# vvvm23/distributed-pytorch-cookbook

Hardware: AMD Instinct MI355X
Metric: tokens/sec (node) GPT-2 training per recipe (DDP/FSDP/PP) at 1/2/4/8 MI355X (higher is better)
Workload: dtype bf16; 1 GPU; model=gpt2-small, global_batch=64, seq_len=1024, parallelism=dp1, recipe=main-ddp.py, reduce_dtype=fp32, pp_comm_dtype=fp32, step_graph=True

## Files before the change

distributed_pytorch_cookbook_amd/ops/csrc/attention.hip:

```cpp
#include "common.h"

#include <cstdlib>
#include <type_traits>

namespace dpc {

struct AttnArgs {
  const void* q; const void* k; const void* v;
  void* o;
  float* lse;
  const unsigned char* pad;
  const void* dout;
  void* dq; void* dk; void* dv;
  float* delta;
  long long ld_qkv, ld_o, ld_dqkv;
  int N, S, H;
  float scale;
  int causal;
  int hd;
  int order;
};

constexpr int KT = 64;
constexpr int QB = 128;
constexpr int NSLOT = 4;
constexpr float LOG2E = 1.4426950408889634f;

template <int HD>
struct AT {
  static_assert(HD == 32 || HD == 64 || HD == 128, "head_dim 32, 64 or 128");
  static constexpr int TILE = KT * HD;
  static constexpr int NPW = HD / 32;
  static constexpr int NST = HD / 16;
  static constexpr int NDT = HD / 32;
};

typedef short4_t __attribute__((address_space(3))) * lds4_t;
typedef __attribute__((address_space(3))) void* lds_void_t;

__device__ __forceinline__ int aswz(int prow) {
  const int a = (prow >> 1) & 7;
  return a ^ ((a & 1) << 2);
}
template <int HD>
__device__ __forceinline__ int toff(int row, int chunk) {
  const int e = row * HD + chunk * 8;
  const int prow = e >> 6, pch = (e >> 3) & 7;
  return (prow << 6) + ((pch ^ aswz(prow)) << 3);
}

__device__ __forceinline__ void dma16(__amdgpu_buffer_rsrc_t rs, int voff, const void* lds) {
  const unsigned la = (unsigned)(uintptr_t)(lds_void_t)lds;
  asm volatile("s_mov_b32 m0, %2\n\ts_nop 0\n\tbuffer_load_dwordx4 %0, %1, 0 offen lds"
               :
               : "v"(voff), "s"(rs), "s"(la)
               : "memory", "m0");
}
__device__ __forceinline__ void dma4(__amdgpu_buffer_rsrc_t rs, int voff, const void* lds) {
  const unsigned la = (unsigned)(uintptr_t)(lds_void_t)lds;
  asm volatile("s_mov_b32 m0, %2\n\ts_nop 0\n\tbuffer_load_dword %0, %1, 0 offen lds"
               :
               : "v"(voff), "s"(rs), "s"(la)
               : "memory", "m0");
}
template <int N>
__device__ __forceinline__ void vm_wait() {
  asm volatile("s_waitcnt vmcnt(%0)" ::"n"(N) : "memory");
}
template <int N>
__device__ __forceinline__ void pin_loaded(const bf16x8 (&x)[N]) {
#pragma unroll
  for (int i = 0; i < N; ++i) asm volatile("" ::"v"(x[i]));
}
__device__ __forceinline__ void pin_loaded(float x) { asm volatile("" ::"v"(x)); }

__device__ __forceinline__ void ring_barrier() {
  __builtin_amdgcn_s_barrier();
  asm volatile("" ::: "memory");
}

__device__ __forceinline__ __amdgpu_buffer_rsrc_t rows_rsrc(const void* base, unsigned ld_bytes, int row0, int S,
                                                           bool valid) {
  const unsigned span = (unsigned)S * ld_bytes;
  const unsigned off = (unsigned)row0 * ld_bytes;
  const unsigned nrec = __builtin_amdgcn_readfirstlane((valid && off < span) ? span - off : 0u);
  return __builtin_amdgcn_make_buffer_rsrc((void*)((const char*)base + off), 0, nrec, 0x00020000);
}

template <int HD>
__device__ __forceinline__ void dma_voff(int (&v)[AT<HD>::NPW], long long ld, int wid, int lane) {
#pragma unroll
  for (int i = 0; i < AT<HD>::NPW; ++i) {
    const int prow = 8 * (wid * AT<HD>::NPW + i) + (lane >> 3);
    const int e = prow * 64 + (((lane & 7) ^ aswz(prow)) << 3);
    const int row = e / HD, chunk = (e % HD) >> 3;
    v[i] = (int)((long long)row * ld * 2 + chunk * 16);
  }
}

template <int HD>
__device__ __forceinline__ void tile_dma(const bf16_t* base, long long ld, int row0, int S, bool valid,
                                         const int (&v)[AT<HD>::NPW], bf16_t* lds, int wid) {
  const __amdgpu_buffer_rsrc_t rs = rows_rsrc(base, (unsigned)(ld * 2), row0, S, valid);
#pragma unroll
  for (int i = 0; i < AT<HD>::NPW; ++i) dma16(rs, v[i], lds + (wid * AT<HD>::NPW + i) * 512);
}

template <int HD>
__device__ __forceinline__ bf16x8 row_frag(const bf16_t* lds, int row0, int st, int lane) {
  return *reinterpret_cast<const bf16x8*>(lds + toff<HD>(row0 + (lane & 31), 2 * st + (lane >> 5)));
}

template <int HD>
__device__ __forceinline__ bf16x8 tr_frag(const bf16_t* lds, int r0, int s, int c0, int lane) {
  const int h = lane >> 5, g2 = (lane >> 4) & 1, i16 = lane & 15, q = i16 >> 2, p = i16 & 3;
  const int row = r0 + 16 * s + 4 * h + q;
  const int col = c0 + 16 * g2 + 4 * p;
  const bf16_t* a0 = lds + toff<HD>(row, col >> 3) + (col & 7);
  const bf16_t* a1 = lds + toff<HD>(row + 8, col >> 3) + (col & 7);
  short4_t lo = __builtin_amdgcn_ds_read_tr16_b64_v4i16((lds4_t)a0);
  short4_t hi = __builtin_amdgcn_ds_read_tr16_b64_v4i16((lds4_t)a1);
  typedef short short8_t __attribute__((ext_vector_type(8)));
  short8_t s8 = {lo[0], lo[1], lo[2], lo[3], hi[0], hi[1], hi[2], hi[3]};
  return __builtin_bit_cast(bf16x8, s8);
}

__device__ __forceinline__ bf16x8 acc_frag(const floatx16& x, int s) {
  uint4 u;
  u.x = pack2bf(x[8 * s + 0], x[8 * s + 1]);
  u.y = pack2bf(x[8 * s + 2], x[8 * s + 3]);
  u.z = pack2bf(x[8 * s + 4], x[8 * s + 5]);
  u.w = pack2bf(x[8 * s + 6], x[8 * s + 7]);
  return __builtin_bit_cast(bf16x8, u);
}

__device__ __forceinline__ int acc_row(int r, int lane) { return (r & 3) + 8 * (r >> 2) + 4 * (lane >> 5); }

__device__ __forceinline__ void store_pair16(bf16_t* row, int g, int hh, uint2 wa, uint2 wb) {
  const auto s0 = __builtin_amdgcn_permlane32_swap(wa.x, wb.x, false, false);
  const auto s1 = __builtin_amdgcn_permlane32_swap(wa.y, wb.y, false, false);
  *reinterpret_cast<uint4*>(row + 8 * g + 8 * hh) = make_uint4(s0[0], s1[0], s0[1], s1[1]);
}

__device__ __forceinline__ float fast_exp2(float x) { return __builtin_amdgcn_exp2f(x); }

__device__ __forceinline__ float max3f(float a, float b, float c) { return fmaxf(fmaxf(a, b), c); }

__device__ __forceinline__ unsigned long long pad_bits(const unsigned char* pad, int k0, int S, int lane) {
  if (!pad) return 0ull;
  const int k = k0 + lane;
  return __ballot(k < S && pad[k] != 0);
}

__device__ __forceinline__ bf16x8 load_row8(const bf16_t* p) {
  return *reinterpret_cast<const bf16x8*>(p);
}

#define MFMA32(a, b, c) __builtin_amdgcn_mfma_f32_32x32x16_bf16((a), (b), (c), 0, 0, 0)

__device__ __forceinline__ void scale16(floatx16& x, float a) {
#pragma unroll
  for (int i = 0; i < 16; ++i) asm volatile("v_mul_f32 %0, %0, %1" : "+v"(x[i]) : "v"(a));
}

template <int K>
__device__ __forceinline__ void zero_if_gt(floatx16& x, int r, int v) {
  asm volatile("v_cmp_lt_i32_e32 vcc, %1, %2\n\tv_cndmask_b32_e64 %0, %0, 0, vcc"
               : "+v"(x[r])
               : "n"(K), "v"(v)
               : "vcc");
}

#define DPC_RS_MUL(i) "v_mul_f32 %" #i ", %" #i ", %16\n\t"
__device__ __forceinline__ void scale16_if(floatx16& x, float a, unsigned long long up) {
  asm volatile(
      "s_cmp_eq_u64 %17, 0\n\t"
      "s_cbranch_scc1 .Ldpc_rs%=\n\t"
      "s_nop 7\n\ts_nop 7\n\t"
      DPC_RS_MUL(0) DPC_RS_MUL(1) DPC_RS_MUL(2) DPC_RS_MUL(3) DPC_RS_MUL(4) DPC_RS_MUL(5) DPC_RS_MUL(6)
      DPC_RS_MUL(7) DPC_RS_MUL(8) DPC_RS_MUL(9) DPC_RS_MUL(10) DPC_RS_MUL(11) DPC_RS_MUL(12)
      DPC_RS_MUL(13) DPC_RS_MUL(14) DPC_RS_MUL(15)
      "s_nop 7\n"
      ".Ldpc_rs%=:"
      : "+v"(x[0]), "+v"(x[1]), "+v"(x[2]), "+v"(x[3]), "+v"(x[4]), "+v"(x[5]), "+v"(x[6]), "+v"(x[7]),
        "+v"(x[8]), "+v"(x[9]), "+v"(x[10]), "+v"(x[11]), "+v"(x[12]), "+v"(x[13]), "+v"(x[14]), "+v"(x[15])
      : "v"(a), "s"(up)
      : "scc");
}
#undef DPC_RS_MUL

#define DPC_RS_MUL(i) "v_mul_f32 %" #i ", %" #i ", %17\n\t"
__device__ __forceinline__ float rescale16_if(floatx16& x, float& m, float& l, float mx, unsigned long long up) {
  float a;
  asm volatile(
      "s_cmp_eq_u64 %20, 0\n\t"
      "s_cbranch_scc1 .Ldpc_ru%=\n\t"
      "s_nop 7\n\ts_nop 7\n\t"
      "v_max_f32 %17, %16, %19\n\t"
      "v_sub_f32 %16, %16, %17\n\t"
      "v_exp_f32 %16, %16\n\t"
      "s_nop 0\n\t"
      "v_swap_b32 %16, %17\n\t"
      "v_mul_f32 %18, %18, %17\n\t"
      DPC_RS_MUL(0) DPC_RS_MUL(1) DPC_RS_MUL(2) DPC_RS_MUL(3) DPC_RS_MUL(4) DPC_RS_MUL(5) DPC_RS_MUL(6)
      DPC_RS_MUL(7) DPC_RS_MUL(8) DPC_RS_MUL(9) DPC_RS_MUL(10) DPC_RS_MUL(11) DPC_RS_MUL(12)
      DPC_RS_MUL(13) DPC_RS_MUL(14) DPC_RS_MUL(15)
      "s_nop 7\n"
      ".Ldpc_ru%=:"
      : "+v"(x[0]), "+v"(x[1]), "+v"(x[2]), "+v"(x[3]), "+v"(x[4]), "+v"(x[5]), "+v"(x[6]), "+v"(x[7]),
        "+v"(x[8]), "+v"(x[9]), "+v"(x[10]), "+v"(x[11]), "+v"(x[12]), "+v"(x[13]), "+v"(x[14]), "+v"(x[15]),
        "+v"(m), "=&v"(a), "+v"(l)
      : "v"(mx), "s"(up)
      : "scc");
  return a;
}
#undef DPC_RS_MUL

__device__ __forceinline__ void zero16(floatx16& x) {
#pragma unroll
  for (int i = 0; i < 16; ++i) x[i] = 0.f;
}

__device__ __forceinline__ int g7_local_attn(int b, int grid) {
  const int xcd = b & 7, q = grid >> 3, r = grid & 7;
  return (xcd < r ? xcd * (q + 1) : r * (q + 1) + (xcd - r) * q) + (b >> 3);
}
__device__ __forceinline__ void work_order1(int nblk, int& bh, int& i) {
  const int nbh = gridDim.x / nblk;
  i = blockIdx.x / nbh;
  bh = blockIdx.x - i * nbh;
}
__device__ __forceinline__ void xcd_work(int nblk, int& bh, int& i) {
  const int b = blockIdx.x, nwg = gridDim.x, xcd = b & 7, q = nwg >> 3, r = nwg & 7;
  const int t = (xcd < r ? xcd * (q + 1) : r * (q + 1) + (xcd - r) * q) + (b >> 3);
  bh = t / nblk;
  i = t - bh * nblk;
}

template <int HD, int OCC>
__global__ __launch_bounds__(256, OCC) void attn_fwd_kernel(AttnArgs p) {
  using A = AT<HD>;
  __shared__ __attribute__((aligned(16))) bf16_t smem[NSLOT * 2 * A::TILE];
  const int S = p.S, H = p.H;
  const int nqb = (S + QB - 1) / QB;
  int bh, bi;
  xcd_work(nqb, bh, bi);
  const int qb = nqb - 1 - bi;
  const int n = bh / H, h = bh % H;
  const int lane = threadIdx.x & 63, hh = lane >> 5;
  const int wid = __builtin_amdgcn_readfirstlane(threadIdx.x >> 6);
  const int q0 = qb * QB + wid * 32;
  const int q = q0 + (lane & 31);
  const long long tok0 = (long long)n * S;
  const bf16_t* Q = static_cast<const bf16_t*>(p.q) + h * HD;
  const bf16_t* K = static_cast<const bf16_t*>(p.k) + tok0 * p.ld_qkv + h * HD;
  const bf16_t* V = static_cast<const bf16_t*>(p.v) + tok0 * p.ld_qkv + h * HD;

  bf16x8 qf[A::NST];
#pragma unroll
  for (int st = 0; st < A::NST; ++st)
    qf[st] = q < S ? load_row8(Q + (tok0 + q) * p.ld_qkv + 16 * st + 8 * hh) : bf16x8{};
  pin_loaded(qf);
  const float c = p.scale * LOG2E;
  const int kend = p.causal ? min(S, qb * QB + QB) : S;
  const int ntiles = (kend + KT - 1) / KT;
  const int last_w = p.causal ? min(ntiles - 1, max(0, min(q0 + 31, S - 1)) / KT) : ntiles - 1;
  const unsigned char* pad = p.pad ? p.pad + (long long)n * S : nullptr;

  int dv[A::NPW];
  dma_voff<HD>(dv, p.ld_qkv, wid, lane);
  auto issue = [&](int t) {
    bf16_t* st = smem + (t % NSLOT) * 2 * A::TILE;
    const bool valid = t < ntiles;
    tile_dma<HD>(K, p.ld_qkv, t * KT, S, valid, dv, st, wid);
    tile_dma<HD>(V, p.ld_qkv, t * KT, S, valid, dv, st + A::TILE, wid);
  };
  auto qk = [&](floatx16 (&s)[2], const bf16_t* lk) {
#pragma unroll
    for (int kb = 0; kb < 2; ++kb) {
      zero16(s[kb]);
#pragma unroll
      for (int st = 0; st < A::NST; ++st)
        s[kb] = MFMA32(row_frag<HD>(lk, kb * 32, st, lane), qf[st], s[kb]);
    }
  };

  float m = -INFINITY, l = 0.f;
  floatx16 o[A::NDT];
#pragma unroll
  for (int d = 0; d < A::NDT; ++d) zero16(o[d]);

  issue(0);
  issue(1);
  issue(2);
  vm_wait<4 * A::NPW>();
  ring_barrier();
  auto step = [&](int t, floatx16 (&sc)[2], floatx16 (&sn)[2]) {
    vm_wait<2 * A::NPW>();
    ring_barrier();
    issue(t + 3);
    const bf16_t* lkn = smem + ((t + 1) % NSLOT) * 2 * A::TILE;
    const bf16_t* lv = smem + (t % NSLOT) * 2 * A::TILE + A::TILE;
    if (t > last_w) return;
    const int kt0 = t * KT;
    const bool need_mask = (p.causal && kt0 + KT - 1 > q0) || (kt0 + KT > S) || pad;
    if (need_mask) {
      const unsigned long long pm = pad_bits(pad, kt0, S, lane);
      const int lim = (p.causal ? min(q, S - 1) : S - 1) - kt0;
#pragma unroll
      for (int kb = 0; kb < 2; ++kb)
#pragma unroll
        for (int r = 0; r < 16; ++r) {
          const int kl = kb * 32 + acc_row(r, lane);
          if (kl > lim || ((pm >> kl) & 1ull)) sc[kb][r] = -INFINITY;
        }
    }
    float mq[4];
#pragma unroll
    for (int q4 = 0; q4 < 4; ++q4) {
      const floatx16& sq = sc[q4 >> 1];
      const int r0 = (q4 & 1) * 8;
      float v = max3f(sq[r0], sq[r0 + 1], sq[r0 + 2]);
      v = max3f(v, sq[r0 + 3], sq[r0 + 4]);
      v = max3f(v, sq[r0 + 5], sq[r0 + 6]);
      mq[q4] = fmaxf(v, sq[r0 + 7]);
    }
    float mx = fmaxf(max3f(mq[0], mq[1], mq[2]), mq[3]);
    mx = fmaxf(mx, __shfl_xor(mx, 32, 64)) * c;
    if (__ballot(mx > m + 8.f)) {
      const float mn = fmaxf(m, mx);
      const float alpha = (mn == -INFINITY) ? 1.f : fast_exp2(m - mn);
      m = mn;
      l *= alpha;
#pragma unroll
      for (int d = 0; d < A::NDT; ++d) scale16(o[d], alpha);
    }
    const float nmu = (m == -INFINITY) ? 0.f : -m;
    qk(sn, lkn);
    float ls = 0.f;
    bf16x8 pb[2][2];
#pragma unroll
    for (int kb = 0; kb < 2; ++kb) {
#pragma unroll
      for (int r = 0; r < 16; ++r) {
        const float e = fast_exp2(fmaf(sc[kb][r], c, nmu));
        sc[kb][r] = e;
        ls += e;
      }
      pb[kb][0] = acc_frag(sc[kb], 0);
      pb[kb][1] = acc_frag(sc[kb], 1);
    }
    l += ls;
#pragma unroll
    for (int kb = 0; kb < 2; ++kb)
#pragma unroll
      for (int ss = 0; ss < 2; ++ss)
#pragma unroll
        for (int d = 0; d < A::NDT; ++d)
          o[d] = MFMA32(tr_frag<HD>(lv, kb * 32, ss, d * 32, lane), pb[kb][ss], o[d]);
  };
  floatx16 s0[2], s1[2];
  qk(s0, smem);
  for (int t = 0; t < ntiles; t += 2) {
    step(t, s0, s1);
    if (t + 1 < ntiles) step(t + 1, s1, s0);
  }
  vm_wait<0>();

  l += __shfl_xor(l, 32, 64);
  if (q < S) {
    const float inv = l > 0.f ? 1.f / l : 0.f;
    bf16_t* O = static_cast<bf16_t*>(p.o) + (tok0 + q) * p.ld_o + h * HD;
#pragma unroll
    for (int d = 0; d < A::NDT; ++d)
#pragma unroll
      for (int g = 0; g < 4; g += 2) {
        uint2 wa, wb;
        wa.x = pack2bf(o[d][4 * g + 0] * inv, o[d][4 * g + 1] * inv);
        wa.y = pack2bf(o[d][4 * g + 2] * inv, o[d][4 * g + 3] * inv);
        wb.x = pack2bf(o[d][4 * g + 4] * inv, o[d][4 * g + 5] * inv);
        wb.y = pack2bf(o[d][4 * g + 6] * inv, o[d][4 * g + 7] * inv);
        store_pair16(O + d * 32, g, hh, wa, wb);
      }
    if (hh == 0) {
      const float lse = (l > 0.f) ? (m + log2f(l)) / LOG2E : INFINITY;
      p.lse[(long long)bh * S + q] = lse;
    }
  }
}

struct PairItem {
  int bh, blk0, blk1, len0, len;
};

template <int HD, int OCC>
__global__ __launch_bounds__(256, OCC) void attn_fwd2_kernel(AttnArgs p, int nitems) {
  using A = AT<HD>;
  __shared__ __attribute__((aligned(16))) bf16_t smem[NSLOT * 2 * A::TILE];
  const int S = p.S, H = p.H;
  const int nqb = (S + QB - 1) / QB;
  const int npr = (nqb + 1) / 2;
  const int grid = gridDim.x;
  const int local = g7_local_attn(blockIdx.x, grid);
  const int lane = threadIdx.x & 63, hh = lane >> 5;
  const int wid = __builtin_amdgcn_readfirstlane(threadIdx.x >> 6);
  auto ntiles_of = [&](int qb) {
    const int kend = p.causal ? min(S, qb * QB + QB) : S;
    return (kend + KT - 1) / KT;
  };
  auto item = [&](int k) {
    PairItem it;
    const int id = local + k * grid;
    it.bh = id / npr;
    const int pr = id - it.bh * npr;
    it.blk0 = nqb - 1 - pr;
    it.blk1 = pr;
    it.len0 = 1 + ntiles_of(it.blk0);
    it.len = it.len0 + (it.blk1 != it.blk0 ? 1 + ntiles_of(it.blk1) : 0);
    return it;
  };
  const int nmine = local < nitems ? (nitems - local + grid - 1) / grid : 0;
  if (nmine == 0) return;
  int total = 0;
  for (int k = 0; k < nmine; ++k) total += item(k).len;

  int dv[A::NPW];
  dma_voff<HD>(dv, p.ld_qkv, wid, lane);
  int is_k = 0, is_off = 0;
  PairItem is_it = item(0);
  long long is_hoff = 0;
  auto enter = [&]() {
    const int n = is_it.bh / H, h = is_it.bh - n * H;
    is_hoff = (long long)n * S * p.ld_qkv + h * HD;
  };
  enter();
  auto issue_next = [&](int e) {
    bf16_t* st = smem + (e % NSLOT) * 2 * A::TILE;
    const bool valid = is_k < nmine;
    const bool second = is_off >= is_it.len0;
    const int i = is_off - (second ? is_it.len0 : 0);
    if (i == 0 || !valid) {
      const bf16_t* base = static_cast<const bf16_t*>(p.q) + is_hoff;
      const int r0 = (second ? is_it.blk1 : is_it.blk0) * QB;
      tile_dma<HD>(base, p.ld_qkv, r0, S, valid, dv, st, wid);
// ... 216 lines not shown
      const int r0 = (second ? is_it.blk1 : is_it.blk0) * QB;
      tile_dma<HD>(base, p.ld_qkv, r0, S, valid, dv, st, wid);
      tile_dma<HD>(base, p.ld_qkv, r0 + KT, S, valid, dv, st + A::TILE, wid);
    } else {
      const bf16_t* K = static_cast<const bf16_t*>(p.k) + is_hoff;
      const bf16_t* V = static_cast<const bf16_t*>(p.v) + is_hoff;
      tile_dma<HD>(K, p.ld_qkv, (i - 1) * KT, S, true, dv, st, wid);
      tile_dma<HD>(V, p.ld_qkv, (i - 1) * KT, S, true, dv, st + A::TILE, wid);
    }
    if (valid && ++is_off == is_it.len) {
      is_off = 0;
      if (++is_k < nmine) {
        is_it = item(is_k);
        enter();
      }
    }
  };
  auto sync = [&](int e) {
    vm_wait<2 * A::NPW>();
    ring_barrier();
    issue_next(e + 3);
  };
  auto slot = [&](int e) -> const bf16_t* { return smem + (e % NSLOT) * 2 * A::TILE; };

  const float c = p.scale * LOG2E;
  bf16x8 qf[A::NST];
  float m = -INFINITY, l = 0.f;
  floatx16 o[A::NDT];
  int q0 = 0, q = 0, last_w = 0;
  int bh = 0, h = 0, n = 0;
  const unsigned char* pad = nullptr;

  auto qk = [&](floatx16 (&s)[2], const bf16_t* lk) {
#pragma unroll
    for (int kb = 0; kb < 2; ++kb) {
      zero16(s[kb]);
#pragma unroll
      for (int st = 0; st < A::NST; ++st) s[kb] = MFMA32(row_frag<HD>(lk, kb * 32, st, lane), qf[st], s[kb]);
    }
  };
  auto finish = [&]() {
    l += __shfl_xor(l, 32, 64);
    if (q < S) {
      const float inv = l > 0.f ? __builtin_amdgcn_rcpf(l) : 0.f;
      bf16_t* O = static_cast<bf16_t*>(p.o) + (long long)n * S * p.ld_o + h * HD + q * (int)p.ld_o;
#pragma unroll
      for (int d = 0; d < A::NDT; ++d)
#pragma unroll
        for (int g = 0; g < 4; g += 2) {
          uint2 wa, wb;
          wa.x = pack2bf(o[d][4 * g + 0] * inv, o[d][4 * g + 1] * inv);
          wa.y = pack2bf(o[d][4 * g + 2] * inv, o[d][4 * g + 3] * inv);
          wb.x = pack2bf(o[d][4 * g + 4] * inv, o[d][4 * g + 5] * inv);
          wb.y = pack2bf(o[d][4 * g + 6] * inv, o[d][4 * g + 7] * inv);
          store_pair16(O + d * 32, g, hh, wa, wb);
        }
      if (hh == 0) p.lse[(long long)bh * S + q] = (l > 0.f) ? (m + log2f(l)) / LOG2E : INFINITY;
    }
  };
  auto tile = [&](auto gen, int e, int t, floatx16 (&sc)[2], floatx16 (&sn)[2]) {
    constexpr bool GEN = decltype(gen)::value;
    const bf16_t* ls = slot(e);
    const bf16_t* lv = ls + A::TILE;
    const int kt0 = t * KT;
    if constexpr (GEN) {
      const bool need_mask = (p.causal && kt0 + KT - 1 > q0) || (kt0 + KT > S) || pad;
      if (need_mask) {
        const int limh = (p.causal ? min(q, S - 1) : S - 1) - kt0 - 4 * hh;
        const unsigned long long pm = pad_bits(pad, kt0, S, lane) >> (4 * hh);
#pragma unroll
        for (int kb = 0; kb < 2; ++kb) {
          const unsigned pk = (unsigned)(pm >> (32 * kb));
#pragma unroll
          for (int r = 0; r < 16; ++r) {
            const int kc = kb * 32 + (r & 3) + 8 * (r >> 2);
            const bool masked = (kc > limh) || ((pk >> ((r & 3) + 8 * (r >> 2))) & 1u);
            if (masked) sc[kb][r] = -INFINITY;
          }
        }
      }
    }
    float mq[4];
#pragma unroll
    for (int q4 = 0; q4 < 4; ++q4) {
      const floatx16& sq = sc[q4 >> 1];
      const int r0 = (q4 & 1) * 8;
      float v = max3f(sq[r0], sq[r0 + 1], sq[r0 + 2]);
      v = max3f(v, sq[r0 + 3], sq[r0 + 4]);
      v = max3f(v, sq[r0 + 5], sq[r0 + 6]);
      mq[q4] = fmaxf(v, sq[r0 + 7]);
    }
    float mx = fmaxf(max3f(mq[0], mq[1], mq[2]), mq[3]);
    {
      const auto sw = __builtin_amdgcn_permlane32_swap(__float_as_uint(mx), __float_as_uint(mx), false, false);
      mx = fmaxf(__uint_as_float(sw[0]), __uint_as_float(sw[1])) * c;
    }
    if constexpr (GEN) {
      if (__ballot(mx > m + 8.f)) {
        const float mn = fmaxf(m, mx);
        const float alpha = (m == -INFINITY) ? 1.f : fast_exp2(m - mn);
        m = mn;
        l *= alpha;
#pragma unroll
        for (int d = 0; d < A::NDT; ++d) scale16(o[d], alpha);
      }
    } else {
      const unsigned long long up = __ballot(mx > m + 8.f);
      const float alpha = rescale16_if(o[0], m, l, mx, up);
#pragma unroll
      for (int d = 1; d < A::NDT; ++d) scale16_if(o[d], alpha, up);
    }
    const float nmu = (!GEN || m != -INFINITY) ? -m : 0.f;
    if constexpr (GEN) {
      if (t + 1 <= last_w) qk(sn, slot(e + 1));
    } else {
      qk(sn, slot(e + 1));
    }
    float lq[4] = {0.f, 0.f, 0.f, 0.f};
    bf16x8 pb[2][2];
#pragma unroll
    for (int kb = 0; kb < 2; ++kb) {
#pragma unroll
      for (int r = 0; r < 16; ++r) {
        const float ex = fast_exp2(fmaf(sc[kb][r], c, nmu));
        sc[kb][r] = ex;
        lq[r & 3] += ex;
      }
      pb[kb][0] = acc_frag(sc[kb], 0);
      pb[kb][1] = acc_frag(sc[kb], 1);
    }
    l += (lq[0] + lq[1]) + (lq[2] + lq[3]);
#pragma unroll
    for (int kb = 0; kb < 2; ++kb)
#pragma unroll
      for (int ss = 0; ss < 2; ++ss)
#pragma unroll
        for (int d = 0; d < A::NDT; ++d)
          o[d] = MFMA32(tr_frag<HD>(lv, kb * 32, ss, d * 32, lane), pb[kb][ss], o[d]);
  };
  using Plain = std::integral_constant<bool, false>;
  using General = std::integral_constant<bool, true>;

  issue_next(0);
  issue_next(1);
  issue_next(2);
  floatx16 sA[2], sB[2];
  int e = 0;
  for (int k = 0; k < nmine; ++k) {
    const PairItem it = item(k);
    for (int half = 0; half < 2; ++half) {
      if (half == 1 && it.blk1 == it.blk0) break;
      const int blk = half ? it.blk1 : it.blk0;
      sync(e);
      const bf16_t* ls = slot(e);
      if (e > 0) finish();
      if (half == 0) {
        bh = it.bh;
        n = bh / H;
        h = bh - n * H;
        pad = p.pad ? p.pad + (long long)n * S : nullptr;
      }
      q0 = blk * QB + wid * 32;
      q = q0 + (lane & 31);
      const int nt = ntiles_of(blk);
      last_w = p.causal ? min(nt - 1, max(0, min(q0 + 31, S - 1)) / KT) : nt - 1;
#pragma unroll
      for (int st = 0; st < A::NST; ++st) qf[st] = row_frag<HD>(ls + (wid >> 1) * A::TILE, 32 * (wid & 1), st, lane);
      m = -INFINITY;
      l = 0.f;
#pragma unroll
      for (int d = 0; d < A::NDT; ++d) zero16(o[d]);
      qk(sA, slot(e + 1));
      ++e;
      int nf = pad ? 0 : min(last_w, S / KT);
      if (p.causal) nf = min(nf, (q0 + 1) / KT);
      int t = 0;
      for (; t + 2 <= nf; t += 2, e += 2) {
        sync(e);
        tile(Plain(), e, t, sA, sB);
        sync(e + 1);
        tile(Plain(), e + 1, t + 1, sB, sA);
      }
      if (t < nf) {
        sync(e);
        tile(Plain(), e, t, sA, sB);
#pragma unroll
        for (int kb = 0; kb < 2; ++kb) sA[kb] = sB[kb];
        ++e;
        ++t;
      }
      for (; t < nt; ++t, ++e) {
        sync(e);
        if (t <= last_w) {
          tile(General(), e, t, sA, sB);
#pragma unroll
          for (int kb = 0; kb < 2; ++kb) sA[kb] = sB[kb];
        }
      }
    }
  }
  finish();
  vm_wait<0>();
}

template <int HD, int OCC, int ABL = 0>
__global__ __launch_bounds__(256, OCC) void attn_bwd_dkdv_kernel(AttnArgs p) {
  using A = AT<HD>;
  __shared__ __attribute__((aligned(16))) bf16_t smem[NSLOT * 2 * A::TILE];
  __shared__ __attribute__((aligned(16))) float srow[NSLOT][2][KT];
  const int S = p.S, H = p.H;
  const int nkb = (S + QB - 1) / QB;
  int bh, kb;
  if (p.order == 1) work_order1(nkb, bh, kb);
  else xcd_work(nkb, bh, kb);
  const int n = bh / H, h = bh % H;
  const int lane = threadIdx.x & 63, hh = lane >> 5;
  const int wid = __builtin_amdgcn_readfirstlane(threadIdx.x >> 6);
  const int k0 = kb * QB + wid * 32;
  const int key = k0 + (lane & 31);
  const long long tok0 = (long long)n * S;
  const bf16_t* Q = static_cast<const bf16_t*>(p.q) + tok0 * p.ld_qkv + h * HD;
  const bf16_t* Kp = static_cast<const bf16_t*>(p.k) + h * HD;
  const bf16_t* Vp = static_cast<const bf16_t*>(p.v) + h * HD;
  const bf16_t* dO = static_cast<const bf16_t*>(p.dout) + tok0 * p.ld_o + h * HD;
  const float* lse = p.delta + (long long)p.N * H * S + (long long)bh * S;
  const float* delta = p.delta + (long long)bh * S;
  const bool key_ok = key < S && !(p.pad && p.pad[(long long)n * S + min(key, S - 1)]);

  bf16x8 kf[A::NST], vf[A::NST];
#pragma unroll
  for (int st = 0; st < A::NST; ++st) {
    kf[st] = bf16x8{};
    vf[st] = bf16x8{};
  }
  const float c = p.scale * LOG2E;
  floatx16 dvt[A::NDT], dkt[A::NDT];
#pragma unroll
  for (int d = 0; d < A::NDT; ++d) {
    zero16(dvt[d]);
    zero16(dkt[d]);
  }

  const int qt_begin = p.causal ? (kb * QB) / KT : 0;
  const int nqt = (S + KT - 1) / KT;
  const int count = nqt - qt_begin;

  int vq[A::NPW], vd[A::NPW];
  dma_voff<HD>(vq, p.ld_qkv, wid, lane);
  dma_voff<HD>(vd, p.ld_o, wid, lane);
  auto issue = [&](int i) {
    const int slot = i % NSLOT, qt = qt_begin + i;
    const bool valid = i < count;
    bf16_t* st = smem + slot * 2 * A::TILE;
    tile_dma<HD>(Q, p.ld_qkv, qt * KT, S, valid, vq, st, wid);
    tile_dma<HD>(dO, p.ld_o, qt * KT, S, valid, vd, st + A::TILE, wid);
    if (wid == 0) {
      dma4(rows_rsrc(lse, 4, qt * KT, S, valid), lane * 4, &srow[slot][0][0]);
      dma4(rows_rsrc(delta, 4, qt * KT, S, valid), lane * 4, &srow[slot][1][0]);
    }
  };
  auto sdp = [&](floatx16& sa, floatx16& dp, const bf16_t* lq, int r0) {
    zero16(sa);
    const float* drow = &srow[((lq - smem) / (2 * A::TILE))][1][0];
#pragma unroll
    for (int g = 0; g < 4; ++g) {
      const float4 d4 = *reinterpret_cast<const float4*>(drow + r0 + 8 * g + 4 * hh);
      dp[4 * g + 0] = d4.x;
      dp[4 * g + 1] = d4.y;
      dp[4 * g + 2] = d4.z;
      dp[4 * g + 3] = d4.w;
    }
#pragma unroll
    for (int st = 0; st < A::NST; ++st) {
      sa = MFMA32(row_frag<HD>(lq, r0, st, lane), kf[st], sa);
      dp = MFMA32(row_frag<HD>(lq + A::TILE, r0, st, lane), vf[st], dp);
    }
  };

  if (count > 0 && !(ABL & 8)) {
    if constexpr (!(ABL & 2)) {
      bf16_t* sk = smem + 2 * 2 * A::TILE;
      bf16_t* sv = smem + 3 * 2 * A::TILE;
      const bf16_t* K0 = Kp + tok0 * p.ld_qkv;
      const bf16_t* V0 = Vp + tok0 * p.ld_qkv;
      tile_dma<HD>(K0, p.ld_qkv, kb * QB, S, true, vq, sk, wid);
      tile_dma<HD>(K0, p.ld_qkv, kb * QB + KT, S, true, vq, sk + A::TILE, wid);
      tile_dma<HD>(V0, p.ld_qkv, kb * QB, S, true, vq, sv, wid);
      tile_dma<HD>(V0, p.ld_qkv, kb * QB + KT, S, true, vq, sv + A::TILE, wid);
    }
    issue(0);
    issue(1);
    if constexpr (!(ABL & 2)) {
      if (wid == 0) vm_wait<4 * A::NPW + 4>();
      else vm_wait<4 * A::NPW>();
      ring_barrier();
      const bf16_t* sk = smem + 2 * 2 * A::TILE + (wid >> 1) * A::TILE;
#pragma unroll
      for (int st = 0; st < A::NST; ++st) {
        kf[st] = row_frag<HD>(sk, 32 * (wid & 1), st, lane);
        vf[st] = row_frag<HD>(sk + 2 * A::TILE, 32 * (wid & 1), st, lane);
      }
      asm volatile("s_waitcnt lgkmcnt(0)" ::: "memory");
      __builtin_amdgcn_sched_barrier(0);
      ring_barrier();
    }
    issue(2);
    if (wid == 0) vm_wait<4 * A::NPW + 4>();
    else vm_wait<4 * A::NPW>();
    ring_barrier();
  }
  auto half = [&](int i, int hf, floatx16& sa, floatx16& dp) {
    const int slot = i % NSLOT;
    const bf16_t* lq = smem + slot * 2 * A::TILE;
    const bf16_t* ldo = lq + A::TILE;
    const int qt0 = (qt_begin + i) * KT;
    const int qs0 = qt0 + 32 * hf;
    const bool active = !(p.causal && qs0 + 31 < k0);
    if (!active) return;
    const bool diag = p.causal && qs0 < k0 + 31;
    sdp(sa, dp, lq, 32 * hf);
    sfor<4>([&](auto G) {
      constexpr int g = decltype(G)::value;
      const float4 l4 = *reinterpret_cast<const float4*>(&srow[slot][0][32 * hf + 8 * g + 4 * hh]);
      const float lv[4] = {l4.x, l4.y, l4.z, l4.w};
#pragma unroll
      for (int e = 0; e < 4; ++e) sa[4 * g + e] = fast_exp2(fmaf(sa[4 * g + e], c, -lv[e]));
    });
    if (diag) {
      const int kd = key - qs0 - 4 * hh;
      sfor<16>([&](auto R) {
        constexpr int r = decltype(R)::value;
        zero_if_gt<8 * (r >> 2) + (r & 3)>(sa, r, kd);
      });
    }
#pragma unroll
    for (int r = 0; r < 16; ++r) dp[r] = sa[r] * dp[r];
#pragma unroll
    for (int ss = 0; ss < 2; ++ss) {
      const bf16x8 pb = acc_frag(sa, ss);
      const bf16x8 db = acc_frag(dp, ss);
#pragma unroll
      for (int d = 0; d < A::NDT; ++d) {
        dvt[d] = MFMA32(tr_frag<HD>(ldo, 32 * hf, ss, d * 32, lane), pb, dvt[d]);
        dkt[d] = MFMA32(tr_frag<HD>(lq, 32 * hf, ss, d * 32, lane), db, dkt[d]);
      }
    }
  };
  floatx16 sa0, dp0, sa1, dp1;
  for (int i = 0; i < ((ABL & 1) ? 0 : count); ++i) {
    if (wid == 0) vm_wait<2 * A::NPW + 2>();
    else vm_wait<2 * A::NPW>();
    ring_barrier();
    issue(i + 3);
    half(i, 0, sa0, dp0);
    half(i, 1, sa1, dp1);
  }
  vm_wait<0>();

  if (key < S && !(ABL & 4)) {
    bf16_t* dK = static_cast<bf16_t*>(p.dk) + (tok0 + key) * p.ld_dqkv + h * HD;
    bf16_t* dV = static_cast<bf16_t*>(p.dv) + (tok0 + key) * p.ld_dqkv + h * HD;
    auto wk = [&](int d, int g) {
      uint2 w = make_uint2(0u, 0u);
      if (key_ok) {
        w.x = pack2bf(dkt[d][4 * g + 0] * p.scale, dkt[d][4 * g + 1] * p.scale);
        w.y = pack2bf(dkt[d][4 * g + 2] * p.scale, dkt[d][4 * g + 3] * p.scale);
      }
      return w;
    };
    auto wv = [&](int d, int g) {
      uint2 u = make_uint2(0u, 0u);
      if (key_ok) {
        u.x = pack2bf(dvt[d][4 * g + 0], dvt[d][4 * g + 1]);
        u.y = pack2bf(dvt[d][4 * g + 2], dvt[d][4 * g + 3]);
      }
      return u;
    };
#pragma unroll
    for (int d = 0; d < A::NDT; ++d)
#pragma unroll
      for (int g = 0; g < 4; g += 2) {
        store_pair16(dK + d * 32, g, hh, wk(d, g), wk(d, g + 1));
        store_pair16(dV + d * 32, g, hh, wv(d, g), wv(d, g + 1));
      }
  }
}

template <int HD, int OCC, int ABL = 0>
__global__ __launch_bounds__(256, OCC) void attn_bwd_dq_kernel(AttnArgs p) {
  using A = AT<HD>;
  __shared__ __attribute__((aligned(16))) bf16_t smem[NSLOT * 2 * A::TILE];
  const int S = p.S, H = p.H;
  const int nqb = (S + QB - 1) / QB;
  int bh, bi;
  if (p.order == 1) work_order1(nqb, bh, bi);
  else xcd_work(nqb, bh, bi);
  const int qb = nqb - 1 - bi;
  const int n = bh / H, h = bh % H;
  const int lane = threadIdx.x & 63, hh = lane >> 5;
  const int wid = __builtin_amdgcn_readfirstlane(threadIdx.x >> 6);
  const int q0 = qb * QB + wid * 32;
  const int q = q0 + (lane & 31);
  const long long tok0 = (long long)n * S;
  const bf16_t* Q = static_cast<const bf16_t*>(p.q) + h * HD;
  const bf16_t* K = static_cast<const bf16_t*>(p.k) + tok0 * p.ld_qkv + h * HD;
  const bf16_t* V = static_cast<const bf16_t*>(p.v) + tok0 * p.ld_qkv + h * HD;
  const bf16_t* dO = static_cast<const bf16_t*>(p.dout) + h * HD;
  const unsigned char* pad = p.pad ? p.pad + (long long)n * S : nullptr;

  bf16x8 qf[A::NST], df[A::NST];
#pragma unroll
  for (int st = 0; st < A::NST; ++st) {
    qf[st] = (q < S && !(ABL & 2)) ? load_row8(Q + (tok0 + q) * p.ld_qkv + 16 * st + 8 * hh) : bf16x8{};
    df[st] = (q < S && !(ABL & 2)) ? load_row8(dO + (tok0 + q) * p.ld_o + 16 * st + 8 * hh) : bf16x8{};
  }
  const float c = p.scale * LOG2E;
  const bf16_t* Op = static_cast<const bf16_t*>(p.o) + h * HD;
  float acc = 0.f;
  if (q < S && !(ABL & 2)) {
#pragma unroll
    for (int st = 0; st < A::NST; ++st) {
      const bf16x8 of = load_row8(Op + (tok0 + q) * p.ld_o + 16 * st + 8 * hh);
      float fo[8], fd[8];
      unpack8(__builtin_bit_cast(uint4, of), fo);
      unpack8(__builtin_bit_cast(uint4, df[st]), fd);
#pragma unroll
      for (int i = 0; i < 8; ++i) acc = fmaf(fo[i], fd[i], acc);
    }
  }
  const float dl = acc + __shfl_xor(acc, 32, 64);
  const float lse2 = q < S ? p.lse[(long long)bh * S + q] * LOG2E : INFINITY;
  if (q < S && hh == 0 && ABL == 0) {
    p.delta[(long long)bh * S + q] = -dl;
    p.delta[(long long)p.N * H * S + (long long)bh * S + q] = lse2;
  }
  pin_loaded(qf);
  pin_loaded(df);
  pin_loaded(lse2);
  pin_loaded(dl);
  floatx16 dqt[A::NDT];
#pragma unroll
  for (int d = 0; d < A::NDT; ++d) zero16(dqt[d]);

  const int kend = p.causal ? min(S, qb * QB + QB) : S;
  const int ntiles = (kend + KT - 1) / KT;

  int dv[A::NPW];
  dma_voff<HD>(dv, p.ld_qkv, wid, lane);
  auto issue = [&](int t) {
    bf16_t* st = smem + (t % NSLOT) * 2 * A::TILE;
    const bool valid = t < ntiles;
    tile_dma<HD>(K, p.ld_qkv, t * KT, S, valid, dv, st, wid);
    tile_dma<HD>(V, p.ld_qkv, t * KT, S, valid, dv, st + A::TILE, wid);
  };
  auto sdp = [&](floatx16& sa, floatx16& dp, const bf16_t* lk, int r0) {
    zero16(sa);
#pragma unroll
    for (int r = 0; r < 16; ++r) dp[r] = -dl;
#pragma unroll
    for (int st = 0; st < A::NST; ++st) {
      sa = MFMA32(row_frag<HD>(lk, r0, st, lane), qf[st], sa);
      dp = MFMA32(row_frag<HD>(lk + A::TILE, r0, st, lane), df[st], dp);
    }
  };

  if (!(ABL & 8)) {
    issue(0);
    issue(1);
    issue(2);
    vm_wait<4 * A::NPW>();
    ring_barrier();
  }
  auto half = [&](int t, int hf, floatx16& sa, floatx16& dp) {
    const bf16_t* lk = smem + (t % NSLOT) * 2 * A::TILE;
    const int kt0 = t * KT;
    const int ks0 = kt0 + 32 * hf;
    const bool active = !(p.causal && ks0 > q0 + 31);
    if (!active) return;
    const bool need_mask = (p.causal && ks0 + 31 > q0) || (ks0 + 32 > S) || pad;
    sdp(sa, dp, lk, 32 * hf);
    if (need_mask) {
      const unsigned long long pm = pad_bits(pad, kt0, S, lane);
      const int lim = (p.causal ? min(q, S - 1) : S - 1) - kt0;
#pragma unroll
      for (int r = 0; r < 16; ++r) {
        const int kl = 32 * hf + acc_row(r, lane);
        float pv = fast_exp2(fmaf(sa[r], c, -lse2));
        pv = (kl > lim || ((pm >> kl) & 1ull)) ? 0.f : pv;
        dp[r] = pv * dp[r];
      }
    } else {
#pragma unroll
      for (int r = 0; r < 16; ++r) dp[r] = fast_exp2(fmaf(sa[r], c, -lse2)) * dp[r];
    }
#pragma unroll
    for (int ss = 0; ss < 2; ++ss) {
      const bf16x8 db = acc_frag(dp, ss);
#pragma unroll
      for (int d = 0; d < A::NDT; ++d)
        dqt[d] = MFMA32(tr_frag<HD>(lk, 32 * hf, ss, d * 32, lane), db, dqt[d]);
    }
  };
  floatx16 sa0, dp0, sa1, dp1;
  for (int t = 0; t < ((ABL & 1) ? 0 : ntiles); ++t) {
    vm_wait<2 * A::NPW>();
    ring_barrier();
    issue(t + 3);
    half(t, 0, sa0, dp0);
    half(t, 1, sa1, dp1);
  }
  vm_wait<0>();

  if (q < S && !(ABL & 4)) {
    bf16_t* dQ = static_cast<bf16_t*>(p.dq) + (tok0 + q) * p.ld_dqkv + h * HD;
#pragma unroll
    for (int d = 0; d < A::NDT; ++d)
#pragma unroll
      for (int g = 0; g < 4; g += 2) {
        uint2 wa, wb;
        wa.x = pack2bf(dqt[d][4 * g + 0] * p.scale, dqt[d][4 * g + 1] * p.scale);
        wa.y = pack2bf(dqt[d][4 * g + 2] * p.scale, dqt[d][4 * g + 3] * p.scale);
        wb.x = pack2bf(dqt[d][4 * g + 4] * p.scale, dqt[d][4 * g + 5] * p.scale);
        wb.y = pack2bf(dqt[d][4 * g + 6] * p.scale, dqt[d][4 * g + 7] * p.scale);
        store_pair16(dQ + d * 32, g, hh, wa, wb);
      }
  }
}

static int launch_fwd(const AttnArgs* a, hipStream_t stream) {
  const int nqb = (a->S + QB - 1) / QB;
  const dim3 blocks((unsigned)(nqb * a->N * a->H));
  const int nitems = ((nqb + 1) / 2) * a->N * a->H;
  const dim3 pairs((unsigned)nitems);
  if (a->hd == 128) hipLaunchKernelGGL((attn_fwd_kernel<128, 1>), blocks, dim3(256), 0, stream, *a);
  else if (a->hd == 64) hipLaunchKernelGGL((attn_fwd3_kernel<64, 2>), pairs, dim3(256), 0, stream, *a, nitems);
  else if (a->S < 512) hipLaunchKernelGGL((attn_fwd2_kernel<32, 2>), pairs, dim3(256), 0, stream, *a, nitems);
  else hipLaunchKernelGGL((attn_fwd3_kernel<32, 2>), pairs, dim3(256), 0, stream, *a, nitems);
  return (int)hipGetLastError();
}

template <int HD, int OCC>
static void launch_bwd_at(const AttnArgs* a, dim3 blocks, hipStream_t stream) {
  hipLaunchKernelGGL((attn_bwd_dq_kernel<HD, OCC>), blocks, dim3(256), 0, stream, *a);
  hipLaunchKernelGGL((attn_bwd_dkdv_kernel<HD, OCC>), blocks, dim3(256), 0, stream, *a);
}
static int launch_bwd(const AttnArgs* a, hipStream_t stream) {
  const dim3 blocks((unsigned)(((a->S + QB - 1) / QB) * a->N * a->H));
  if (a->hd == 128) launch_bwd_at<128, 1>(a, blocks, stream);
  else if (a->hd == 64) launch_bwd_at<64, 2>(a, blocks, stream);
  else launch_bwd_at<32, 3>(a, blocks, stream);
  return (int)hipGetLastError();
}

}

using namespace dpc;

static bool attn_args_ok(const AttnArgs* a, bool bwd) {
  if (a->hd != 32 && a->hd != 64 && a->hd != 128) return false;
  if (a->N <= 0 || a->S <= 0 || a->H <= 0) return false;
  if (a->ld_qkv % 8 || a->ld_o % 8 || (bwd && a->ld_dqkv % 8)) return false;
  const long long ld = a->ld_qkv > a->ld_o ? a->ld_qkv : a->ld_o;
  if (((long long)a->S + 256) * ld * 2 >= 0xffffffffll) return false;
  return true;
}

DPC_API int dpc_attn_fwd(const AttnArgs* a, hipStream_t stream) {
  if (!attn_args_ok(a, false)) return (int)hipErrorInvalidValue;
  return launch_fwd(a, stream);
}

template <int ABL>
static void attn_lab_launch(const AttnArgs* a, int which, hipStream_t stream) {
  dim3 grid((unsigned)(((a->S + QB - 1) / QB) * a->N * a->H));
  if (which == 1) hipLaunchKernelGGL((attn_bwd_dkdv_kernel<64, 2, ABL>), grid, dim3(256), 0, stream, *a);
  else hipLaunchKernelGGL((attn_bwd_dq_kernel<64, 2, ABL>), grid, dim3(256), 0, stream, *a);
}
DPC_API int dpc_attn_bwd_lab(const AttnArgs* a, int which, int abl, hipStream_t stream) {
  if (!attn_args_ok(a, true) || a->hd != 64) return (int)hipErrorInvalidValue;
  if (which != 1 && which != 2) return (int)hipErrorInvalidValue;
  switch (abl) {
    case 0: attn_lab_launch<0>(a, which, stream); break;
    case 1: attn_lab_launch<1>(a, which, stream); break;
    case 2: attn_lab_launch<2>(a, which, stream); break;
    case 4: attn_lab_launch<4>(a, which, stream); break;
    case 6: attn_lab_launch<6>(a, which, stream); break;
    case 3: attn_lab_launch<3>(a, which, stream); break;
    case 5: attn_lab_launch<5>(a, which, stream); break;
    case 7: attn_lab_launch<7>(a, which, stream); break;
    case 15: attn_lab_launch<15>(a, which, stream); break;
    default: return (int)hipErrorInvalidValue;
  }
  return (int)hipGetLastError();
}


static int g_attn_order = -1;
static int attn_order() {
  if (g_attn_order < 0) g_attn_order = getenv("DPC_ATTN_ORDER") ? atoi(getenv("DPC_ATTN_ORDER")) : 1;
  return g_attn_order;
}
DPC_API void dpc_attn_set_order(int v) { g_attn_order = v; }

DPC_API int dpc_attn_bwd(const AttnArgs* a_in, hipStream_t stream) {
  AttnArgs b = *a_in;
  b.order = attn_order();
  const AttnArgs* a = &b;
  if (!attn_args_ok(a, true)) return (int)hipErrorInvalidValue;
  return launch_bwd(a, stream);
}
```

Before: 1.019 million tokens/s.

## Stage dQ-kernel Q/dO/O loads via LDS DMA and coalesce dK/dV stores

The dq backward kernel now loads Q, dO and O tiles through asynchronous LDS DMA alongside the K/V ring prologue, instead of doing per-lane global row loads. Fragments are then read from shared memory, and the delta/lse writes move to the epilogue. The dkv kernel, for head dim 64, stages dK/dV through swizzled shared memory and writes whole rows, and its prologue wait/barrier ordering is adjusted. This is meant to overlap prologue latency and get coalesced stores, at the cost of more LDS per block (which may lower occupancy) and extra barriers.

New measurement: 1.025 million tokens/s, median of 6. No clear change (+0.6%).

```diff
diff --git a/distributed_pytorch_cookbook_amd/ops/csrc/attention.hip b/distributed_pytorch_cookbook_amd/ops/csrc/attention.hip
--- a/distributed_pytorch_cookbook_amd/ops/csrc/attention.hip
+++ b/distributed_pytorch_cookbook_amd/ops/csrc/attention.hip
@@ -140,6 +140,28 @@
   const auto s0 = __builtin_amdgcn_permlane32_swap(wa.x, wb.x, false, false);
   const auto s1 = __builtin_amdgcn_permlane32_swap(wa.y, wb.y, false, false);
   *reinterpret_cast<uint4*>(row + 8 * g + 8 * hh) = make_uint4(s0[0], s1[0], s0[1], s1[1]);
+}
+
+template <int HD>
+__device__ __forceinline__ int oswz(int row) {
+  return (HD >= 64 ? row : row >> 1) & (HD / 8 - 1);
+}
+template <int HD>
+__device__ __forceinline__ void stage_pair16(bf16_t* blk, int row, int chunk, int hh, uint2 wa, uint2 wb) {
+  const auto s0 = __builtin_amdgcn_permlane32_swap(wa.x, wb.x, false, false);
+  const auto s1 = __builtin_amdgcn_permlane32_swap(wa.y, wb.y, false, false);
+  *reinterpret_cast<uint4*>(blk + row * HD + (((chunk + hh) ^ oswz<HD>(row)) << 3)) =
+      make_uint4(s0[0], s1[0], s0[1], s1[1]);
+}
+template <int HD>
+__device__ __forceinline__ void store_rows(bf16_t* g, long long ld, int nrows, const bf16_t* blk, int lane) {
+  constexpr int CH = HD / 8;
+#pragma unroll
+  for (int j = 0; j < CH / 2; ++j) {
+    const int idx = j * 64 + lane, row = idx / CH, ch = idx % CH;
+    const uint4 v = *reinterpret_cast<const uint4*>(blk + row * HD + ((ch ^ oswz<HD>(row)) << 3));
+    if (row < nrows) *reinterpret_cast<uint4*>(g + row * ld + ch * 8) = v;
+  }
 }
 
 __device__ __forceinline__ float fast_exp2(float x) { return __builtin_amdgcn_exp2f(x); }
@@ -962,12 +984,11 @@
       }
       asm volatile("s_waitcnt lgkmcnt(0)" ::: "memory");
       __builtin_amdgcn_sched_barrier(0);
-      ring_barrier();
-    }
+    }
+    if (wid == 0) vm_wait<2 * A::NPW + 2>();
+    else vm_wait<2 * A::NPW>();
+    ring_barrier();
     issue(2);
-    if (wid == 0) vm_wait<4 * A::NPW + 4>();
-    else vm_wait<4 * A::NPW>();
-    ring_barrier();
   }
   auto half = [&](int i, int hf, floatx16& sa, floatx16& dp) {
     const int slot = i % NSLOT;
@@ -1017,9 +1038,12 @@
   }
   vm_wait<0>();
 
-  if (key < S && !(ABL & 4)) {
-    bf16_t* dK = static_cast<bf16_t*>(p.dk) + (tok0 + key) * p.ld_dqkv + h * HD;
-    bf16_t* dV = static_cast<bf16_t*>(p.dv) + (tok0 + key) * p.ld_dqkv + h * HD;
+  constexpr bool LINES = HD == 64;
+  if constexpr (!(ABL & 4)) {
+    if constexpr (LINES) ring_barrier();
+    bf16_t* bk = smem + wid * 64 * HD;
+    bf16_t* bv = bk + 32 * HD;
+    const int row = lane & 31;
     auto wk = [&](int d, int g) {
       uint2 w = make_uint2(0u, 0u);
       if (key_ok) {
@@ -1040,16 +1064,30 @@
     for (int d = 0; d < A::NDT; ++d)
 #pragma unroll
       for (int g = 0; g < 4; g += 2) {
-        store_pair16(dK + d * 32, g, hh, wk(d, g), wk(d, g + 1));
-        store_pair16(dV + d * 32, g, hh, wv(d, g), wv(d, g + 1));
-      }
+        if constexpr (LINES) {
+          stage_pair16<HD>(bk, row, 4 * d + g, hh, wk(d, g), wk(d, g + 1));
+          stage_pair16<HD>(bv, row, 4 * d + g, hh, wv(d, g), wv(d, g + 1));
+        } else if (key < S) {
+          bf16_t* dK = static_cast<bf16_t*>(p.dk) + (tok0 + key) * p.ld_dqkv + h * HD;
+          bf16_t* dV = static_cast<bf16_t*>(p.dv) + (tok0 + key) * p.ld_dqkv + h * HD;
+          store_pair16(dK + d * 32, g, hh, wk(d, g), wk(d, g + 1));
+          store_pair16(dV + d * 32, g, hh, wv(d, g), wv(d, g + 1));
+        }
+      }
+    if constexpr (LINES) {
+      __builtin_amdgcn_wave_barrier();
+      bf16_t* dK = static_cast<bf16_t*>(p.dk) + (tok0 + k0) * p.ld_dqkv + h * HD;
+      bf16_t* dV = static_cast<bf16_t*>(p.dv) + (tok0 + k0) * p.ld_dqkv + h * HD;
+      store_rows<HD>(dK, p.ld_dqkv, S - k0, bk, lane);
+      store_rows<HD>(dV, p.ld_dqkv, S - k0, bv, lane);
+    }
   }
 }
 
 template <int HD, int OCC, int ABL = 0>
 __global__ __launch_bounds__(256, OCC) void attn_bwd_dq_kernel(AttnArgs p) {
   using A = AT<HD>;
-  __shared__ __attribute__((aligned(16))) bf16_t smem[NSLOT * 2 * A::TILE];
+  __shared__ __attribute__((aligned(16))) bf16_t smem[(NSLOT + 1) * 2 * A::TILE];
   const int S = p.S, H = p.H;
   const int nqb = (S + QB - 1) / QB;
   int bh, bi;
@@ -1071,33 +1109,10 @@
   bf16x8 qf[A::NST], df[A::NST];
 #pragma unroll
   for (int st = 0; st < A::NST; ++st) {
-    qf[st] = (q < S && !(ABL & 2)) ? load_row8(Q + (tok0 + q) * p.ld_qkv + 16 * st + 8 * hh) : bf16x8{};
-    df[st] = (q < S && !(ABL & 2)) ? load_row8(dO + (tok0 + q) * p.ld_o + 16 * st + 8 * hh) : bf16x8{};
+    qf[st] = bf16x8{};
+    df[st] = bf16x8{};
   }
   const float c = p.scale * LOG2E;
-  const bf16_t* Op = static_cast<const bf16_t*>(p.o) + h * HD;
-  float acc = 0.f;
-  if (q < S && !(ABL & 2)) {
-#pragma unroll
-    for (int st = 0; st < A::NST; ++st) {
-      const bf16x8 of = load_row8(Op + (tok0 + q) * p.ld_o + 16 * st + 8 * hh);
-      float fo[8], fd[8];
-      unpack8(__builtin_bit_cast(uint4, of), fo);
-      unpack8(__builtin_bit_cast(uint4, df[st]), fd);
-#pragma unroll
-      for (int i = 0; i < 8; ++i) acc = fmaf(fo[i], fd[i], acc);
-    }
-  }
-  const float dl = acc + __shfl_xor(acc, 32, 64);
-  const float lse2 = q < S ? p.lse[(long long)bh * S + q] * LOG2E : INFINITY;
-  if (q < S && hh == 0 && ABL == 0) {
-    p.delta[(long long)bh * S + q] = -dl;
-    p.delta[(long long)p.N * H * S + (long long)bh * S + q] = lse2;
-  }
-  pin_loaded(qf);
-  pin_loaded(df);
-  pin_loaded(lse2);
-  pin_loaded(dl);
   floatx16 dqt[A::NDT];
 #pragma unroll
   for (int d = 0; d < A::NDT; ++d) zero16(dqt[d]);
@@ -1105,8 +1120,32 @@
   const int kend = p.causal ? min(S, qb * QB + QB) : S;
   const int ntiles = (kend + KT - 1) / KT;
 
+  constexpr int ROWP = (ABL & 2) ? 0 : 6 * A::NPW;
+  constexpr int RINGP = (ABL & 8) ? 0 : 4 * A::NPW;
+  float ndl = -0.f, lse2, lse_q;
+  [[maybe_unused]] bf16x8 of[A::NST];
+  {
+    const float* lp = p.lse + (long long)bh * S + min(q, S - 1);
+    asm volatile("global_load_dword %0, %1, off" : "=&v"(lse_q) : "v"(lp) : "memory");
+  }
   int dv[A::NPW];
   dma_voff<HD>(dv, p.ld_qkv, wid, lane);
+  if constexpr (ROWP != 0) {
+    int dvo[A::NPW];
+    dma_voff<HD>(dvo, p.ld_o, wid, lane);
+    const bf16_t* Q0 = Q + tok0 * p.ld_qkv;
+    const bf16_t* dO0 = dO + tok0 * p.ld_o;
+    const bf16_t* O0 = static_cast<const bf16_t*>(p.o) + tok0 * p.ld_o + h * HD;
+    bf16_t* sq = smem + 2 * 2 * A::TILE;
+    bf16_t* sd = smem + 3 * 2 * A::TILE;
+    bf16_t* so = smem + NSLOT * 2 * A::TILE;
+    tile_dma<HD>(Q0, p.ld_qkv, qb * QB, S, true, dv, sq, wid);
+    tile_dma<HD>(Q0, p.ld_qkv, qb * QB + KT, S, true, dv, sq + A::TILE, wid);
+    tile_dma<HD>(dO0, p.ld_o, qb * QB, S, true, dvo, sd, wid);
+    tile_dma<HD>(dO0, p.ld_o, qb * QB + KT, S, true, dvo, sd + A::TILE, wid);
+    tile_dma<HD>(O0, p.ld_o, qb * QB, S, true, dvo, so, wid);
+    tile_dma<HD>(O0, p.ld_o, qb * QB + KT, S, true, dvo, so + A::TILE, wid);
+  }
   auto issue = [&](int t) {
     bf16_t* st = smem + (t % NSLOT) * 2 * A::TILE;
     const bool valid = t < ntiles;
@@ -1116,7 +1155,7 @@
   auto sdp = [&](floatx16& sa, floatx16& dp, const bf16_t* lk, int r0) {
     zero16(sa);
 #pragma unroll
-    for (int r = 0; r < 16; ++r) dp[r] = -dl;
+    for (int r = 0; r < 16; ++r) dp[r] = ndl;
 #pragma unroll
     for (int st = 0; st < A::NST; ++st) {
       sa = MFMA32(row_frag<HD>(lk, r0, st, lane), qf[st], sa);
@@ -1124,13 +1163,47 @@
     }
   };
 
-  if (!(ABL & 8)) {
+  if constexpr (RINGP != 0) {
     issue(0);
     issue(1);
+  }
+  vm_wait<RINGP>();
+  asm volatile("" : "+v"(lse_q));
+  lse2 = q < S ? lse_q * LOG2E : INFINITY;
+  if constexpr (ROWP != 0) {
+    ring_barrier();
+    const bf16_t* sq = smem + 2 * 2 * A::TILE + (wid >> 1) * A::TILE;
+    const int r0 = 32 * (wid & 1);
+#pragma unroll
+    for (int st = 0; st < A::NST; ++st) {
+      qf[st] = row_frag<HD>(sq, r0, st, lane);
+      df[st] = row_frag<HD>(sq + 2 * A::TILE, r0, st, lane);
+      of[st] = row_frag<HD>(sq + (NSLOT - 2) * 2 * A::TILE, r0, st, lane);
+    }
+    asm volatile("s_waitcnt lgkmcnt(0)" ::: "memory");
+    __builtin_amdgcn_sched_barrier(0);
+  }
+  if constexpr (RINGP != 0) {
+    vm_wait<2 * A::NPW>();
+    ring_barrier();
     issue(2);
-    vm_wait<4 * A::NPW>();
-    ring_barrier();
-  }
+  }
+  if constexpr (ROWP != 0) {
+    float acc = 0.f;
+#pragma unroll
+    for (int st = 0; st < A::NST; ++st) {
+      float fo[8], fd[8];
+      unpack8(__builtin_bit_cast(uint4, of[st]), fo);
+      unpack8(__builtin_bit_cast(uint4, df[st]), fd);
+#pragma unroll
+      for (int i = 0; i < 8; ++i) acc = fmaf(fo[i], fd[i], acc);
+    }
+    ndl = -(acc + __shfl_xor(acc, 32, 64));
+    pin_loaded(qf);
+    pin_loaded(df);
+    pin_loaded(ndl);
+  }
+  pin_loaded(lse2);
   auto half = [&](int t, int hf, floatx16& sa, floatx16& dp) {
     const bf16_t* lk = smem + (t % NSLOT) * 2 * A::TILE;
     const int kt0 = t * KT;
@@ -1140,7 +1213,9 @@
     const bool need_mask = (p.causal && ks0 + 31 > q0) || (ks0 + 32 > S) || pad;
     sdp(sa, dp, lk, 32 * hf);
     if (need_mask) {
-      const unsigned long long pm = pad_bits(pad, kt0, S, lane);
+      int lz = lane;
+      asm volatile("" : "+v"(lz));
+      const unsigned long long pm = pad_bits(pad, kt0, S, lz);
       const int lim = (p.causal ? min(q, S - 1) : S - 1) - kt0;
 #pragma unroll
       for (int r = 0; r < 16; ++r) {
@@ -1171,8 +1246,15 @@
   }
   vm_wait<0>();
 
-  if (q < S && !(ABL & 4)) {
-    bf16_t* dQ = static_cast<bf16_t*>(p.dq) + (tok0 + q) * p.ld_dqkv + h * HD;
+  int le = lane;
+  asm volatile("" : "+v"(le));
+  const int qe = q0 + (le & 31), hhe = le >> 5;
+  if (qe < S && hhe == 0 && ABL == 0) {
+    p.delta[(long long)bh * S + qe] = ndl;
+    p.delta[(long long)p.N * H * S + (long long)bh * S + qe] = lse2;
+  }
+  if (qe < S && !(ABL & 4)) {
+    bf16_t* dQ = static_cast<bf16_t*>(p.dq) + (tok0 + qe) * p.ld_dqkv + h * HD;
 #pragma unroll
     for (int d = 0; d < A::NDT; ++d)
 #pragma unroll
@@ -1182,7 +1264,7 @@
         wa.y = pack2bf(dqt[d][4 * g + 2] * p.scale, dqt[d][4 * g + 3] * p.scale);
         wb.x = pack2bf(dqt[d][4 * g + 4] * p.scale, dqt[d][4 * g + 5] * p.scale);
         wb.y = pack2bf(dqt[d][4 * g + 6] * p.scale, dqt[d][4 * g + 7] * p.scale);
-        store_pair16(dQ + d * 32, g, hh, wa, wb);
+        store_pair16(dQ + d * 32, g, hhe, wa, wb);
       }
   }
 }
```
